# routineLife1/DRBA

Hardware: AMD Instinct MI355X
Metric: interpolated frames/sec @1080p RIFE x2 (higher is better)
Workload: dtype f32 (2xfp16-term MFMA operands = 22 significand bits, fp32 accumulate)

## Files before the change

### drba_amd/_lib.py

```python
import ctypes as C
import os

_HERE = os.path.dirname(os.path.abspath(__file__))
LIB_PATH = os.path.join(_HERE, "csrc", "libdrba_hip.so")
HEADER_PATH = os.path.join(os.path.dirname(_HERE), "include", "drba_hip.h")


def _header_abi_version():
    import re
    if not os.path.exists(HEADER_PATH):
        return None
    with open(HEADER_PATH) as f:
        m = re.search(r"^#define\s+DRBA_ABI_VERSION\s+(\d+)", f.read(), flags=re.M)
    if m is None:
        raise RuntimeError(f"{HEADER_PATH} does not define DRBA_ABI_VERSION")
    return int(m.group(1))


ABI_VERSION = _header_abi_version()

_p = C.c_void_p
_i = C.c_int
_f = C.c_float
_d = C.c_double
# ... 1 lines not shown


class ConvLayer(C.Structure):
    _fields_ = [("packed_w", C.c_void_p), ("bias", C.c_void_p), ("beta", C.c_void_p), ("cin", C.c_int), ("cout", C.c_int),
                ("stride", C.c_int), ("act", C.c_int), ("cfg", C.c_int), ("residual", C.c_int), ("deconv", C.c_int),
                ("pixel_shuffle", C.c_int)]


SIGNATURES = {
    "drba_abi_version": (_i, []),
    "drba_rife_splat_ws_floats": (_z, [_i, _i, _i, _i]),
    "drba_set_range_check": (_i, [_i]),
    "drba_status_word": (_i, [C.POINTER(C.c_void_p)]),
    "drba_status_clear": (_i, []),
    "drba_stream_create_cu_mask": (_i, [C.POINTER(C.c_uint32), _i, C.POINTER(C.c_void_p)]),
    "drba_stream_destroy": (_i, [_p]),
    "drba_conv_state_reset": (_i, [_p]),
    "drba_trace_begin": (_i, []),
    "drba_trace_end": (_i, []),
    "drba_trace_resume": (_i, []),
    "drba_trace_count": (_i, []),
    "drba_trace_get": (_i, [_i, C.POINTER(C.c_char_p), C.POINTER(C.c_uint), C.POINTER(C.c_float)]),
    "drba_trace_get_start": (_i, [_i, C.POINTER(C.c_float), C.POINTER(C.c_ulonglong)]),
    "drba_error_string": (C.c_char_p, [_i]),
    "drba_softsplat": (_i, [_p, _p, _p, _p, _p, _i, _i, _i, _i, _i, _i, _p]),
    "drba_softsplat_ws_floats": (_z, [_i, _i, _i, _i]),
    "drba_softsplat_again": (_i, [_p, _p, _p, _i, _i, _i, _i, _i, _i, _p]),
    "drba_quad_interleave": (_i, [_p, _p, _i, _i, _i, _i, _p]),
    "drba_softsplat_index": (_i, [_p, _p, _p, _i, _i, _i, _i, _p]),
    "drba_softsplat_gather_quad": (_i, [_p, _p, _p, _i, _i, _i, _i, _i, _i, _p]),
    "drba_backwarp": (_i, [_p, _p, _p, _i, _i, _i, _i, _i, _p]),
    "drba_flow_distance": (_i, [_p, _p, _i, _i, _i, _p]),
    "drba_flow_reverse": (_i, [_p, _p, _p, _i, _i, _i, _p]),
    "drba_drm_rife_linear": (_i, [_p, _p, _f, _p, _f, _p, _p, _i, _i, _i, _p]),
    "drba_drm_rife_linear_batch": (_i, [_p, _i, _f, _p, _i, _i, _p]),
    "drba_drm_ratio": (_i, [_p, _p, _f, _p, _p, _i, _i, _i, _p]),
    "drba_affine": (_i, [_p, _f, _f, _p, _z, _p]),
    "drba_mul_map": (_i, [_p, _p, _p, _i, _i, _i, _i, _p]),
    "drba_fill_holes": (_i, [_p, _p, _p, _p, _z, _p]),
    "drba_drm_retime": (_i, [_p, _p, _d, _d, _z, _p]),
    "drba_resize_bilinear": (_i, [_p, _p, _i, _i, _i, _i, _i, _f, _f, _p]),
    "drba_u8hwc_to_f32nchw": (_i, [_p, _p, _i, _i, _p]),
    "drba_f32nchw_to_u8hwc": (_i, [_p, _p, _i, _i, _p]),
    "drba_to_inp": (_i, [_p, _p, _i, _i, _i, _i, _f, _f, _p]),
    "drba_to_inp_x4": (_i, [_p, _p, _p, _i, _i, _i, _i, _f, _f, _p]),
    "drba_to_out": (_i, [_p, _p, _i, _i, _i, _i, _f, _f, _i, _p]),
    "drba_u16hwc_to_f32nchw": (_i, [_p, _p, _i, _i, _f, _p]),
    "drba_f32nchw_to_u16hwc": (_i, [_p, _p, _i, _i, _f, _p]),
    "drba_to_inp16_x4": (_i, [_p, _p, _p, _i, _i, _i, _i, _f, _f, _f, _p]),
    "drba_to_out16": (_i, [_p, _p, _i, _i, _i, _i, _f, _f, _i, _f, _p]),
    "drba_ssim3d_32": (_i, [_p, _p, _p, _p]),
    "drba_ssim3d_ws_floats": (_z, [_i, _i, _i]),
    "drba_ssim3d": (_i, [_p, _p, _p, _p, _i, _i, _i, _i, _d, _p]),
    "drba_frame_error_ws_floats": (_z, [_i, _z]),
    "drba_frame_error_u8": (_i, [_p, _p, _p, _p, _i, _z, _p]),
    "drba_frame_error_f32": (_i, [_p, _p, _p, _p, _i, _z, _p]),
    "drba_frame_error_u16_ws_floats": (_z, [_i, _z]),
    "drba_frame_error_u16": (_i, [_p, _p, _p, _p, _i, _z, _p]),
    "drba_conv3x3_pick_cfg": (_i, [_i, _i, _i, _i, _i]),
    "drba_conv3x3_num_cfgs": (_i, []),
    "drba_conv3x3_cfg_stride": (_i, [_i]),
    "drba_conv3x3_cfg_family": (_i, [_i]),
    "drba_deconv4x4_cfg_family": (_i, [_i]),
    "drba_deconv4x4_num_cfgs": (_i, []),
    "drba_conv3x3_packed_floats": (_z, [_i, _i, _i]),
    "drba_conv3x3_pack": (_i, [_p, _p, _i, _i, _i]),
# ... 126 lines not shown
```

### drba_amd/csrc/common.hpp

```cpp
#pragma once
#include <hip/hip_runtime.h>
#include <hip/hip_ext.h>
#include <stdint.h>
#include <stdlib.h>

#include "../../include/drba_hip.h"

#define DRBA_CHECK_LAUNCH()                                   \
  do {                                                        \
    if (hipGetLastError() != hipSuccess) return DRBA_ELAUNCH; \
  } while (0)

namespace drba {

struct TimedLaunch {
  hipEvent_t start, stop;
};
extern bool g_trace_on;
TimedLaunch trace_launch(const void *host_fn, const char *fallback_name, dim3 grid, hipStream_t stream);

#define DRBA_LAUNCH(kernel, grid, block, lds, stream, ...)                                                     \
  do {                                                                                                         \
    if (drba::g_trace_on) {                                                                                    \
      const drba::TimedLaunch tl_ = drba::trace_launch((const void *)(kernel), #kernel, grid, stream);         \
// ... 172 lines not shown
__device__ __forceinline__ void sample_x4(const float *__restrict__ px, int W, const Taps &t, float (&v)[3]) {
  const int xb = min(t.x0, W - 2);
  const bool edge = t.x0 != xb;
  const f32x4v a0 = *reinterpret_cast<const f32x4v *>(px + ((size_t)t.y0 * W + xb) * 4), a1 = *reinterpret_cast<const f32x4v *>(px + ((size_t)t.y0 * W + xb + 1) * 4);
  const f32x4v b0 = *reinterpret_cast<const f32x4v *>(px + ((size_t)t.y1 * W + xb) * 4), b1 = *reinterpret_cast<const f32x4v *>(px + ((size_t)t.y1 * W + xb + 1) * 4);
#pragma unroll
  for (int c = 0; c < 3; ++c) {
    const float al = edge ? a1[c] : a0[c], bl = edge ? b1[c] : b0[c];
    v[c] = al * t.wnw + a1[c] * t.wne + bl * t.wsw + b1[c] * t.wse;
  }
}

struct Lerp {
  int i0, i1;
  float w0, w1;
};
__device__ __forceinline__ Lerp lerp_src(int dst, float scale, int size) {
  float s = scale * ((float)dst + 0.5f) - 0.5f;
  if (s < 0.f) s = 0.f;
  Lerp l;
  l.i0 = min((int)s, size - 1);
  l.i1 = l.i0 + (l.i0 < size - 1 ? 1 : 0);
  l.w1 = s - (float)l.i0;
  l.w0 = 1.f - l.w1;
  return l;
}

__device__ __forceinline__ float lerp2_fma(float wy0, float wy1, float wx0, float wx1, float p00, float p01, float p10, float p11) {
  const float top = __fmaf_rn(wx0, p00, __fmul_rn(wx1, p01));
  const float bot = __fmaf_rn(wx0, p10, __fmul_rn(wx1, p11));
  return __fmaf_rn(wy0, top, __fmul_rn(wy1, bot));
}

}
```

### drba_amd/csrc/ifnet_glue.hip

```cpp
#include "common.hpp"
#include "flow_terms.hpp"

#include <string.h>

#include <stdlib.h>

using namespace drba;

namespace {

__device__ __forceinline__ Lerp lerp_src_aten(int dst, float scale, int size) {
  float s = __fmaf_rn(scale, (float)dst + 0.5f, -0.5f);
  if (s < 0.f) s = 0.f;
  Lerp l;
  l.i0 = min((int)s, size - 1);
  l.i1 = l.i0 + (l.i0 < size - 1 ? 1 : 0);
  l.w1 = __fsub_rn(s, (float)l.i0);
  l.w0 = __fsub_rn(1.f, l.w1);
  return l;
}
__device__ __forceinline__ float lerp2_aten(const Lerp &ly, const Lerp &lx, float a, float b, float c, float d) {
  const float top = __fmaf_rn(lx.w0, a, __fmul_rn(lx.w1, b));
  const float bot = __fmaf_rn(lx.w0, c, __fmul_rn(lx.w1, d));
  return __fmaf_rn(ly.w0, top, __fmul_rn(ly.w1, bot));
// ... 845 lines not shown
  const float m = 1.f / (1.f + expf(-mk));
  if (img0x) {
    float a[3], b[3];
    sample_x4(img0x, W, t0, a);
    sample_x4(img1x, W, t1, b);
#pragma unroll
    for (int c = 0; c < 3; ++c) out[(size_t)c * P + p] = a[c] * m + b[c] * (1.f - m);
    return;
  }
#pragma unroll
  for (int c = 0; c < 3; ++c) {
    const float a = sample(img0 + (size_t)c * P, W, t0), b = sample(img1 + (size_t)c * P, W, t1);
    out[(size_t)c * P + p] = a * m + b * (1.f - m);
  }
}

__global__ void __launch_bounds__(256)
ifblock_update_kernel(const UpdateItems items, float *__restrict__ mask, float *__restrict__ feat, int h, int w, int H, int W,
                      float scale, float inv_scale) {
  const float *__restrict__ tmp = items.tmp[blockIdx.y];
  const float *flow_in = items.flow_in[blockIdx.y];
  float *flow_out = items.flow_out[blockIdx.y];
  const size_t P = (size_t)H * W, p_lo = (size_t)h * w;
  const int nch = (mask || feat) ? 13 : 4;
  const Tile2D tp_ = tile_pixel(W, H);
  if (tp_.valid) {
    const int y = tp_.y, x = tp_.x;
    const size_t p = (size_t)y * W + x;
    const Lerp ly = lerp_src(y, inv_scale, h), lx = lerp_src(x, inv_scale, w);
    const size_t o00 = (size_t)ly.i0 * w + lx.i0, o01 = (size_t)ly.i0 * w + lx.i1;
    const size_t o10 = (size_t)ly.i1 * w + lx.i0, o11 = (size_t)ly.i1 * w + lx.i1;
    for (int c = 0; c < nch; ++c) {
      const float *t = tmp + (size_t)c * p_lo;
      const float top = lx.w0 * t[o00] + lx.w1 * t[o01];
      const float bot = lx.w0 * t[o10] + lx.w1 * t[o11];
      const float v = ly.w0 * top + ly.w1 * bot;
      if (c < 4) {
        const float fd = v * scale;
        flow_out[(size_t)c * P + p] = flow_in ? flow_in[(size_t)c * P + p] + fd : fd;
      } else if (c == 4) {
        if (mask) mask[p] = v;
      } else if (feat) {
        feat[(size_t)(c - 5) * P + p] = v;
      }
    }
  }
}

__global__ void __launch_bounds__(256)
warp_blend_kernel(const float *__restrict__ img0, const float *__restrict__ img1, const float *__restrict__ flow,
                  const float *__restrict__ mask_lo, int h, int w, float inv_scale, float *__restrict__ out, int H,
                  int W) {
  const size_t P = (size_t)H * W;
  const Tile2D tp_ = tile_pixel(W, H);
  if (tp_.valid) {
    const int y = tp_.y, x = tp_.x;
    const size_t p = (size_t)y * W + x;
    const Taps t0 = taps_border(warp_coord(x, W, flow[p]), warp_coord(y, H, flow[P + p]), W, H);
    const Taps t1 = taps_border(warp_coord(x, W, flow[2 * P + p]), warp_coord(y, H, flow[3 * P + p]), W, H);
    const Lerp ly = lerp_src(y, inv_scale, h), lx = lerp_src(x, inv_scale, w);
    const float top = lx.w0 * mask_lo[(size_t)ly.i0 * w + lx.i0] + lx.w1 * mask_lo[(size_t)ly.i0 * w + lx.i1];
    const float bot = lx.w0 * mask_lo[(size_t)ly.i1 * w + lx.i0] + lx.w1 * mask_lo[(size_t)ly.i1 * w + lx.i1];
    const float mk = ly.w0 * top + ly.w1 * bot;
    const float m = 1.f / (1.f + expf(-mk));
#pragma unroll
    for (int c = 0; c < 3; ++c) {
      const float a = sample(img0 + (size_t)c * P, W, t0), b = sample(img1 + (size_t)c * P, W, t1);
      out[(size_t)c * P + p] = a * m + b * (1.f - m);
    }
  }
}

}
// ... 360 lines not shown
```

### drba_amd/csrc/splat_warp.hip

```cpp
#include "common.hpp"

#include <string.h>

using namespace drba;

namespace {

template <bool ZEROS>
__global__ void __launch_bounds__(256) backwarp_kernel(const float *__restrict__ in, const float *__restrict__ flow,
                                float *__restrict__ out, int C, int H, int W) {
  const int n = blockIdx.y;
  const size_t P = (size_t)H * W;
  in += (size_t)n * C * P;
  flow += (size_t)n * 2 * P;
  out += (size_t)n * C * P;
  for (size_t p = (size_t)blockIdx.x * blockDim.x + threadIdx.x; p < P; p += (size_t)gridDim.x * blockDim.x) {
    const int y = (int)(p / W), x = (int)(p - (size_t)y * W);
    const float sx = warp_coord(x, W, flow[p]), sy = warp_coord(y, H, flow[P + p]);
    if (!ZEROS) {
      const Taps t = taps_border(sx, sy, W, H);
      for (int c = 0; c < C; ++c) out[(size_t)c * P + p] = sample(in + (size_t)c * P, W, t);
    } else {
      const float fx = floorf(sx), fy = floorf(sy);
      const int x0 = (int)fx, y0 = (int)fy;
      const float wx1 = sx - fx, wy1 = sy - fy, wx0 = 1.f - wx1, wy0 = 1.f - wy1;
      const bool okx0 = x0 >= 0 && x0 < W, okx1 = x0 + 1 >= 0 && x0 + 1 < W;
      const bool oky0 = y0 >= 0 && y0 < H, oky1 = y0 + 1 >= 0 && y0 + 1 < H;
      const bool fin = isfinite(sx) && isfinite(sy);
      for (int c = 0; c < C; ++c) {
        const float *pl = in + (size_t)c * P;
        float v = 0.f;
        if (fin) {
          if (okx0 && oky0) v += pl[(size_t)y0 * W + x0] * (wx0 * wy0);
          if (okx1 && oky0) v += pl[(size_t)y0 * W + x0 + 1] * (wx1 * wy0);
// ... 123 lines not shown
    if (x >= W || y >= H) continue;
    const size_t p = (size_t)y * W + x;
    const SplatSrc<MODE> s = splat_source<MODE>(fs, fo, P, p, x, y, t, eps);
    if (!s.finite) continue;
    if (s.is_short) {
      const int rx = s.fx < 0.f ? (int)ceilf(-s.fx) : (int)floorf(s.fx) + 2;
      const int ry = s.fy < 0.f ? (int)ceilf(-s.fy) : (int)floorf(s.fy) + 2;
      r = max(r, max(rx, ry));
      continue;
    }
    if (MODE == 0) {
      const float v[2] = {s.v[0], s.v[1]};
      scatter_avg<2>(gacc, x, y, s.fx, s.fy, v, H, W, dirty, tiles_x);
    } else {
      const float v[1] = {s.v[0]};
      scatter_avg<1>(gacc, x, y, s.fx, s.fy, v, H, W, dirty, tiles_x);
    }
  }
  if ((size_t)gridDim.z * tiles > (size_t)kReachWords) return;
  __shared__ int wr[4];
#pragma unroll
  for (int d = 32; d >= 1; d >>= 1) r = max(r, __shfl_xor(r, d, 64));
  if ((tid & 63) == 0) wr[tid >> 6] = r;
  __syncthreads();
  if (tid == 0) reach[(size_t)n * tiles + blockIdx.y * tiles_x + blockIdx.x] = max(max(wr[0], wr[1]), max(wr[2], wr[3]));
}

constexpr int kSX = 32, kSY = 16;
static_assert(kRMax <= kSY, "the reach map reads the 3 x 3 tiles around an output tile: a halo may not span more than one tile (DRBA_SPLAT_R)");
constexpr int kKX = kSX + 1, kKY = kSY + 1;
constexpr int kNKEY = kKX * kKY;
constexpr int kCAP = 1536;

template <int MODE, int R>
__device__ __forceinline__ void splat_tile_body(const float *__restrict__ fs, const float *__restrict__ fo, float t, float eps,
                                                float *gacc, int *dirty, float *__restrict__ out, int H, int W, int *cnt,
                                                int *wsum, float4 *rec, int *spilled_) {
  constexpr int NV = MODE == 0 ? 2 : 1;
  constexpr int kSWX = kSX + 2 * R, kSWY = kSY + 2 * R;
  constexpr int kSPT = (kSWX * kSWY + 255) / 256;
  constexpr int kR = R;
  volatile int &spilled = *spilled_;
  const size_t P = (size_t)H * W;
  const int was_dirty = __builtin_nontemporal_load(dirty);
  const int tx0 = blockIdx.x * kSX, ty0 = blockIdx.y * kSY;
  const int tid = threadIdx.x;
  for (int i = tid; i <= kNKEY; i += 256) cnt[i] = 0;
  if (tid == 0) spilled = 0;
  __syncthreads();

  float raw[kSPT][MODE == 0 ? 2 : 4];
#pragma unroll
  for (int i = 0; i < kSPT; ++i) {
    const int e = min(tid + i * 256, kSWX * kSWY - 1);
    const int ry = e / kSWX, rx = e - ry * kSWX;
    const int y = min(max(ty0 - kR + ry, 0), H - 1), x = min(max(tx0 - kR + rx, 0), W - 1);
    const size_t p = (size_t)y * W + x;
    raw[i][0] = fs[p];
    raw[i][1] = fs[P + p];
    if (MODE != 0) {
      raw[i][2] = fo[p];
      raw[i][3] = fo[P + p];
    }
  }
  int kr[kSPT];
  float4 val[kSPT];
#pragma unroll
  for (int i = 0; i < kSPT; ++i) {
    kr[i] = -1;
    const int e = tid + i * 256;
    const int ry = e / kSWX, rx = e - ry * kSWX;
    const int y = ty0 - kR + ry, x = tx0 - kR + rx;
    if (e >= kSWX * kSWY || x < 0 || x >= W || y < 0 || y >= H) continue;
    const SplatSrc<MODE> sp = splat_source_from<MODE>(raw[i][0], raw[i][1], MODE == 0 ? 0.f : raw[i][2],
                                                      MODE == 0 ? 0.f : raw[i][3], x, y, t, eps);
    if (!sp.finite || !sp.is_short) continue;
    const float X = (float)x + sp.fx, Y = (float)y + sp.fy;
    const int kx = (int)floorf(X) - tx0 + 1, ky = (int)floorf(Y) - ty0 + 1;
    if (kx < 0 || kx >= kKX || ky < 0 || ky >= kKY) continue;
    const int key = ky * kKX + kx;
    kr[i] = (key << 16) | (atomicAdd(&cnt[key], 1) & 0xFFFF);
    val[i] = make_float4(sp.v[0], sp.v[1], X - (float)tx0, Y - (float)ty0);
  }
  __syncthreads();

  {
    constexpr int PER = (kNKEY + 255) / 256;
    int v[PER], tot = 0;
#pragma unroll
    for (int j = 0; j < PER; ++j) {
      const int k = tid * PER + j;
      v[j] = k < kNKEY ? cnt[k] : 0;
      tot += v[j];
    }
    int inc = tot;
#pragma unroll
    for (int d = 1; d < 64; d <<= 1) {
      const int o = __shfl_up(inc, d, 64);
      if ((tid & 63) >= d) inc += o;
    }
    if ((tid & 63) == 63) wsum[tid >> 6] = inc;
    __syncthreads();
    int run = inc - tot;
    for (int w = 0; w < (tid >> 6); ++w) run += wsum[w];
#pragma unroll
    for (int j = 0; j < PER; ++j) {
// ... 55 lines not shown
        const float wy = dy ? Y - fl_y : (fl_y + 1.f) - Y;
        const float w = wx * wy;
        a0 += r.x * w;
        if (NV == 2) a1 += r.y * w;
        sw += w;
      }
    }
    const size_t p = (size_t)y * W + x;
    float g0 = 0.f, g1 = 0.f, gw = 0.f;
    if (collect) {
      float *g = gacc + p * (NV + 1);
      g0 = g[0], g1 = NV == 2 ? g[1] : 0.f, gw = g[NV];
      if (g0 != 0.f || g1 != 0.f || gw != 0.f) {
        g[0] = 0.f;
        if (NV == 2) g[1] = 0.f;
        g[NV] = 0.f;
      }
    }
    sw += gw;
    const float nrm = sw + 0.0000001f;
    const bool gap = (sw / nrm) < 0.999f;
    if (MODE == 0) {
      a0 += g0;
      a1 += g1;
      out[p] = (gap ? fill : -1.f * (a0 / nrm)) * 2.f;
      out[P + p] = (gap ? fill : -1.f * (a1 / nrm)) * 2.f;
    } else {
      a0 += g0;
      float o = a0 / nrm;
      if (gap) o = splat_source<MODE>(fs, fo, P, p, x, y, t, eps).v[0];
      out[p] = o;
    }
  }
}

template <int MODE>
__global__ void __launch_bounds__(256) splat_tiled(const float *__restrict__ fs, const float *__restrict__ fo, float t,
                                                   const float *__restrict__ t_dev, float eps, float *ws,
                                                   float *__restrict__ out, int H, int W, const SplatJobs jobs) {
  constexpr int NV = MODE == 0 ? 2 : 1;
  if (t_dev) t = *t_dev;
  __shared__ int cnt[kNKEY + 1];
  __shared__ int wsum[4];
  __shared__ float4 rec[kCAP];
  __shared__ int spilled;
  static_assert(kSX == 32 && kSY == 16, "scatter_avg and the pre-pass work on 32 x 16 tiles");
  const int n = blockIdx.z;
  const size_t P = (size_t)H * W;
  if (jobs.n) {
    fs = jobs.fs[n], fo = jobs.fo[n], t = jobs.t[n], out = jobs.out[n];
  } else {
    fs += (size_t)n * 2 * P;
    if (fo) fo += (size_t)n * 2 * P;
    out += (size_t)n * (MODE == 0 ? 2 : 1) * P;
  }
  const int tiles_x = gridDim.x, tiles_y = gridDim.y, tiles = tiles_x * tiles_y;
  const int *reach = reinterpret_cast<const int *>(ws) + (size_t)n * tiles;
  float *gacc = ws + kReachWords;
  int *dirty = reinterpret_cast<int *>(gacc + (size_t)gridDim.z * P * (NV + 1)) + ((size_t)n * tiles_y + blockIdx.y) * tiles_x + blockIdx.x;
  gacc += (size_t)n * P * (NV + 1);
  int r = kRMax;
  if ((size_t)gridDim.z * tiles <= (size_t)kReachWords) {
    r = 0;
    const int bx = blockIdx.x, by = blockIdx.y;
#pragma unroll
    for (int dy = -1; dy <= 1; ++dy)
#pragma unroll
      for (int dx = -1; dx <= 1; ++dx) {
        const int yy = by + dy, xx = bx + dx;
        if (yy >= 0 && yy < tiles_y && xx >= 0 && xx < tiles_x) r = max(r, __builtin_nontemporal_load(reach + yy * tiles_x + xx));
      }
    r = __builtin_amdgcn_readfirstlane(r);
  }
  if (r <= 4) splat_tile_body<MODE, 4>(fs, fo, t, eps, gacc, dirty, out, H, W, cnt, wsum, rec, &spilled);
  else if (r <= 8) splat_tile_body<MODE, 8>(fs, fo, t, eps, gacc, dirty, out, H, W, cnt, wsum, rec, &spilled);
  else splat_tile_body<MODE, kRMax>(fs, fo, t, eps, gacc, dirty, out, H, W, cnt, wsum, rec, &spilled);
}


constexpr int kChunk = 16, kScanPerBlock = 4096;

struct __attribute__((aligned(16))) SplatRec {
  int src;
  float X, Y;
  float m;
};

__device__ __forceinline__ float splat_weight_1d(float X, float fl, int d) { return d ? X - fl : (fl + 1.f) - X; }

__device__ __forceinline__ long long splat_key(const float *__restrict__ flow, size_t P, size_t p, int x, int y, int H, int W,
                                               float &X, float &Y) {
  X = (float)x + flow[p];
  Y = (float)y + flow[P + p];
  if (!(isfinite(X) && isfinite(Y))) return -1;
  const float fx = floorf(X), fy = floorf(Y);
  if (fx < -1.f || fx > (float)(W - 1) || fy < -1.f || fy > (float)(H - 1)) return -1;
  return (long long)((int)fy + 1) * (W + 1) + ((int)fx + 1);
}

__global__ void __launch_bounds__(256) splat_sort_count(const float *__restrict__ flow, int *__restrict__ cnt, int H, int W) {
  const int n = blockIdx.y;
  const size_t P = (size_t)H * W, Pk = (size_t)(H + 1) * (W + 1);
  flow += (size_t)n * 2 * P;
  cnt += (size_t)n * Pk;
  for (size_t p = (size_t)blockIdx.x * blockDim.x + threadIdx.x; p < P; p += (size_t)gridDim.x * blockDim.x) {
    const int y = (int)(p / W), x = (int)(p - (size_t)y * W);
    float X, Y;
    const long long k = splat_key(flow, P, p, x, y, H, W, X, Y);
    if (k >= 0) atomicAdd(&cnt[k], 1);
// ... 350 lines not shown
  else
    DRBA_LAUNCH(backwarp_kernel<true>, g, dim3(kBlock), 0, (hipStream_t)stream, in, flow, out, C, H, W);
  DRBA_CHECK_LAUNCH();
  return DRBA_OK;
}

int drba_flow_distance(const float *flow, float *out, int N, int H, int W, void *stream) {
  if (!flow || !out || N <= 0 || H <= 0 || W <= 0) return DRBA_EINVAL;
  dim3 g(grid_for((size_t)H * W), N);
  DRBA_LAUNCH(distance_kernel, g, dim3(kBlock), 0, (hipStream_t)stream, flow, out, H, W);
  DRBA_CHECK_LAUNCH();
  return DRBA_OK;
}

size_t drba_rife_splat_ws_floats(int N, int H, int W, int values) {
  if (N <= 0 || H <= 0 || W <= 0 || values < 1 || values > 2) return 0;
  return (size_t)kReachWords + (size_t)N * H * W * (values + 1) + (size_t)N * ((W + kSX - 1) / kSX) * ((H + kSY - 1) / kSY);
}

int drba_flow_reverse(const float *flow, float *out, float *ws, int N, int H, int W, void *stream) {
  if (!flow || !out || !ws || N <= 0 || H <= 0 || W <= 0) return DRBA_EINVAL;
  hipStream_t s = (hipStream_t)stream;
  SplatJobs none;
  none.n = 0;
  dim3 g((W + kSX - 1) / kSX, (H + kSY - 1) / kSY, N);
  DRBA_LAUNCH(splat_long_prepass<0>, g, dim3(kBlock), 0, s, flow, (const float *)nullptr, 0.f,
                     (const float *)nullptr, 0.f, ws, H, W, none);
  DRBA_LAUNCH(splat_tiled<0>, g, dim3(kBlock), 0, s, flow, (const float *)nullptr, 0.f, (const float *)nullptr,
                     0.f, ws, out, H, W, none);
  DRBA_CHECK_LAUNCH();
  return DRBA_OK;
}

int drba_drm_rife_linear(const float *flow_self, const float *flow_other, float t, const float *t_dev, float eps,
                         float *out, float *ws, int N, int H, int W, void *stream) {
  if (!flow_self || !flow_other || !out || !ws || N <= 0 || H <= 0 || W <= 0) return DRBA_EINVAL;
  hipStream_t s = (hipStream_t)stream;
  SplatJobs none;
  none.n = 0;
  dim3 g((W + kSX - 1) / kSX, (H + kSY - 1) / kSY, N);
  DRBA_LAUNCH(splat_long_prepass<1>, g, dim3(kBlock), 0, s, flow_self, flow_other, t, t_dev,
                     eps, ws, H, W, none);
  DRBA_LAUNCH(splat_tiled<1>, g, dim3(kBlock), 0, s, flow_self, flow_other, t, t_dev, eps, ws, out, H, W, none);
  DRBA_CHECK_LAUNCH();
  return DRBA_OK;
}

int drba_drm_rife_linear_batch(const drba_drm_job_t *jobs, int n_jobs, float eps, float *ws, int H, int W, void *stream) {
  if (!jobs || n_jobs <= 0 || n_jobs > DRBA_MAX_STAGE_ITEMS || !ws || H <= 0 || W <= 0) return DRBA_EINVAL;
  SplatJobs J;
  memset(&J, 0, sizeof(J));
  J.n = n_jobs;
  for (int k = 0; k < n_jobs; ++k) {
    if (!jobs[k].flow_self || !jobs[k].flow_other || !jobs[k].out) return DRBA_EINVAL;
    J.fs[k] = jobs[k].flow_self, J.fo[k] = jobs[k].flow_other, J.t[k] = jobs[k].t, J.out[k] = jobs[k].out;
  }
  hipStream_t s = (hipStream_t)stream;
  dim3 g((W + kSX - 1) / kSX, (H + kSY - 1) / kSY, n_jobs);
  DRBA_LAUNCH(splat_long_prepass<1>, g, dim3(kBlock), 0, s, J.fs[0], J.fo[0], 0.f, (const float *)nullptr, eps, ws,
              H, W, J);
  DRBA_LAUNCH(splat_tiled<1>, g, dim3(kBlock), 0, s, J.fs[0], J.fo[0], 0.f, (const float *)nullptr, eps, ws, J.out[0], H, W, J);
  DRBA_CHECK_LAUNCH();
  return DRBA_OK;
}

int drba_drm_ratio(const float *flow10, const float *flow12, float eps, float *drm10, float *drm12, int N, int H,
// ... 39 lines not shown
```

### drba_amd/models/rife.py

```python
import os

import numpy as np
import torch

from drba_amd import handoff, ops as _ops
from drba_amd.models.lookahead import Lookahead, shared_stream
from drba_amd.models.lookahead import split as split_lookahead
from drba_amd.models.drm import calc_drm_rife
from drba_amd.models.rife_426_heavy.IFNet_HDv3 import IFNet
from drba_amd.models.utils.tools import convert, load_weights


class RIFE:
    supports_lookahead = True
    STAT_KEYS = ("groups_formed", "staged_groups", "group_collects", "groups_dropped", "single_steps", "encoder_prefetch_hits",
                 "encoder_prefetch_misses", "pairflow_prefetch_hits", "lookahead_hits")
    stats = None

    def _count(self, key):
        if self.stats is None:
            self.stats = dict.fromkeys(self.STAT_KEYS, 0)
        self.stats[key] += 1
    _look = None

# ... 30 lines not shown
                if f0 is None:
                    f0, f1 = self._encoded(I0), self._encoded(I1)
                output.append(len(items))
                items.append((I0, I1, float(t), f0, f1))
        return self._fill(output, items)

    def _fill(self, output, items):
        if items:
            frames = self.ifnet.forward_pairs(items, self.scale_list)
            output = [frames[o] if isinstance(o, int) else o for o in output]
        return output

    def calc_flow(self, a, b, f0=None, f1=None):
        _, _, H, W = a.shape
        f0 = self._encoded(a) if f0 is None else f0
        f1 = self._encoded(b) if f1 is None else f1
        s = self.scale_list[0]
        xin = _ops.ifblock_input(a, b, f0, f1, 0.5, None, None, 1.0, s)
        flow = _ops.ifblock_update(self.ifnet.block[0].core(xin), None, H, W, s)
        rev = _ops.flow_reverse(flow.reshape(2, 2, H, W))
        flow01, flow10 = rev[0:1], rev[1:2]
        if _ops.PAIR_FEATURES and f0.is_cuda:
            _ops.pair_interleaved(f0)
            _ops.pair_interleaved(f1)
        return flow01, flow10, f0, f1

    def calc_flow_batch(self, pairs):
        B = len(pairs)
        _, _, H, W = pairs[0][0].shape
        s = self.scale_list[0]
        h, w = int(np.floor(H * (1.0 / s))), int(np.floor(W * (1.0 / s)))
        xin = torch.empty((B, 39, h, w), dtype=torch.float32, device=pairs[0][0].device)
        _ops.stage_inputs([(a, b, 0.5, fa, fb) for a, b, fa, fb in pairs], None, None, 1.0, s, xin, lds=False)
        flow = _ops.flow_updates(self.ifnet.block[0].core(xin), [None] * B, H, W, s, whole=True)
        rev = _ops.flow_reverse(flow.reshape(2 * B, 2, H, W))
        out = []
        for k, (a, b, fa, fb) in enumerate(pairs):
            if _ops.PAIR_FEATURES:
                _ops.pair_interleaved(fa)
                _ops.pair_interleaved(fb)
            out.append((rev[2 * k:2 * k + 1], rev[2 * k + 1:2 * k + 2], fa, fb))
        return out

    def _group_flows(self, F, n, fa):
        P, todo = [None] * n, []
        for j in range(n):
            a, b = F[j + 1], F[j + 2]
            if handoff.peek(b, "_drba_pairflow", handoff.token_of(self), a) is not None:
                P[j] = self._pair_flow(a, b, None)
            else:
                todo.append(j)
        if todo:
            feats = {}
            for j in todo:
                for x in (F[j + 1], F[j + 2]):
                    if id(x) not in feats:
                        feats[id(x)] = fa if (x is F[1] and fa is not None) else self._encoded(x)
            res = self.calc_flow_batch([(F[j + 1], F[j + 2], feats[id(F[j + 1])], feats[id(F[j + 2])]) for j in todo])
            for j, r in zip(todo, res):
                P[j] = r
        return P

    def intake_stream(self, device):
        if self.ENC_ON_MAIN:
            return None
        if getattr(self, "_enc_stream", None) is None:
            self._enc_stream = shared_stream(device, "prefetch")
        return self._enc_stream
# ... 207 lines not shown
```

### drba_amd/ops.py

```python
import ctypes as C
import math
import os

import numpy as np
import torch

from drba_amd import _lib
from drba_amd import tunecache as _tunecache

_MODES = {"sum": 0, "avg": 1, "linear": 2, "soft": 3}
_EPS = {None: 0, "addeps": 0, "zeroeps": 1, "clipeps": 2}


def default_device():
    if not torch.cuda.is_available():
        raise _lib.DrbaHipError("drba_amd needs an MI355X (no GPU visible and there is no CPU fallback)")
    return torch.device("cuda", torch.cuda.current_device())


_raw_stream = getattr(torch._C, "_cuda_getCurrentRawStream", None)


def _stream():
    if _raw_stream is not None:
# ... 213 lines not shown
                       "drba_softsplat_again")
        res.append(out)
    return res


def backwarp(x, flow, padding="border"):
    x, flow = _f32(x, "input"), _f32(flow, "flow")
    n, c, h, w = x.shape
    out = torch.empty_like(x)
    _lib.check(_lib.load().drba_backwarp(_p(x), _p(flow), _p(out), n, c, h, w, 0 if padding == "border" else 1,
                                         _stream()), "drba_backwarp")
    return out


def flow_distance(flow):
    flow = _f32(flow, "flow")
    n, _, h, w = flow.shape
    out = torch.empty((n, 1, h, w), dtype=torch.float32, device=flow.device)
    _lib.check(_lib.load().drba_flow_distance(_p(flow), _p(out), n, h, w, _stream()), "drba_flow_distance")
    return out


def flow_reverse(flow):
    flow = _f32(flow, "flow")
    n, _, h, w = flow.shape
    out = torch.empty_like(flow)
    ws = _zero_workspace(flow.device, _lib.load().drba_rife_splat_ws_floats(n, h, w, 2))
    first = _trace_pos()
    _lib.check(_lib.load().drba_flow_reverse(_p(flow), _p(out), _p(ws), n, h, w, _stream()), "drba_flow_reverse")
    _tag(first, [None, (16.0 * n * h * w, "byte", f"flow_reverse {(n, h, w)}")])
    return out


def drm_rife_linear(flow_self, flow_other, t, eps=1e-4, t_dev=None):
    a, b = _f32(flow_self, "flow_self"), _f32(flow_other, "flow_other")
    n, _, h, w = a.shape
    out = torch.empty((n, 1, h, w), dtype=torch.float32, device=a.device)
    ws = _zero_workspace(a.device, _lib.load().drba_rife_splat_ws_floats(n, h, w, 1))
    first = _trace_pos()
    _lib.check(_lib.load().drba_drm_rife_linear(_p(a), _p(b), float(t), _p(t_dev), float(eps), _p(out), _p(ws), n, h,
                                                w, _stream()), "drba_drm_rife_linear")
    _tag(first, [None, (20.0 * n * h * w, "byte", f"drm_rife_linear {(n, h, w)}")])
    return out


def drm_rife_linear_many(jobs, eps=1e-4):
    if not jobs:
        return []
    flows = [(_f32(a, "flow_self"), _f32(b, "flow_other"), float(t)) for a, b, t in jobs]
    _, _, h, w = flows[0][0].shape
    dev = flows[0][0].device
    res = []
    for c0 in range(0, len(flows), _lib.MAX_STAGE_ITEMS):
        chunk = flows[c0:c0 + _lib.MAX_STAGE_ITEMS]
        n = len(chunk)
        out = torch.empty((n, 1, h, w), dtype=torch.float32, device=dev)
        arr = (_lib.DrmJob * n)()
        for k, (a, b, t) in enumerate(chunk):
            if tuple(a.shape) != (1, 2, h, w) or tuple(b.shape) != (1, 2, h, w):
                raise _lib.DrbaHipError("drm_rife_linear_many: every flow must be [1,2,H,W] of one size")
            arr[k].flow_self, arr[k].flow_other, arr[k].t, arr[k].out = a.data_ptr(), b.data_ptr(), t, out[k].data_ptr()
        ws = _zero_workspace(dev, _lib.load().drba_rife_splat_ws_floats(n, h, w, 1))
        first = _trace_pos()
        _lib.check(_lib.load().drba_drm_rife_linear_batch(C.cast(arr, C.c_void_p), n, float(eps), _p(ws), h, w, _stream()),
                   "drba_drm_rife_linear_batch")
        _tag(first, [None, (20.0 * n * h * w, "byte", f"drm_rife_linear {(n, h, w)}")])
# ... 1258 lines not shown
```

### include/drba_hip.h

```cpp
#ifndef DRBA_HIP_H
#define DRBA_HIP_H

#include <stddef.h>
#include <stdint.h>

#ifdef __cplusplus
extern "C" {
#endif

#define DRBA_OK 0
#define DRBA_EINVAL (-1)
#define DRBA_EUNSUPPORTED (-2)
#define DRBA_ELAUNCH (-3)

#define DRBA_ABI_VERSION 12
int drba_abi_version(void);
const char *drba_error_string(int code);
int drba_set_range_check(int on);
#define DRBA_STATUS_CONV_SPLIT 0
#define DRBA_STATUS_CONV_DMA 1
#define DRBA_STATUS_CONV_KS 2
#define DRBA_STATUS_LINEAR 3
#define DRBA_STATUS_ATTENTION 4
#define DRBA_STATUS_STAGE 5
#define DRBA_STATUS_HEAD 6
int drba_status_word(volatile unsigned long long **host_word);
int drba_status_clear(void);

int drba_conv_state_reset(void *stream);
int drba_stream_create_cu_mask(const uint32_t *mask, int words, void **stream);
int drba_stream_destroy(void *stream);

int drba_trace_begin(void);
int drba_trace_end(void);
int drba_trace_resume(void);
int drba_trace_count(void);
int drba_trace_get(int i, const char **name, unsigned *grid3, float *ms);
int drba_trace_get_start(int i, float *ms_since_first, unsigned long long *stream);

int drba_softsplat(const float *in, const float *flow, const float *metric, float *out, float *ws,
                   int N, int C, int H, int W, int mode, int eps, void *stream);
size_t drba_softsplat_ws_floats(int N, int C, int H, int W);
int drba_softsplat_again(const float *in, float *out, float *ws, int N, int C, int H, int W, int mode, int eps, void *stream);
int drba_quad_interleave(const float *in, float *out, int N, int C, int H, int W, void *stream);
int drba_softsplat_index(const float *flow, const float *metric, float *ws, int N, int H, int W, int mode, void *stream);
int drba_softsplat_gather_quad(const float *in_quad, float *out, float *ws, int N, int C, int H, int W, int mode, int eps,
                               void *stream);

int drba_backwarp(const float *in, const float *flow, float *out, int N, int C, int H, int W,
                  int padding, void *stream);

int drba_flow_distance(const float *flow, float *out, int N, int H, int W, void *stream);

size_t drba_rife_splat_ws_floats(int N, int H, int W, int values);
int drba_flow_reverse(const float *flow, float *out, float *ws, int N, int H, int W, void *stream);

int drba_drm_rife_linear(const float *flow_self, const float *flow_other, float t, const float *t_dev,
                         float eps, float *out, float *ws, int N, int H, int W, void *stream);
typedef struct drba_drm_job {
  const float *flow_self, *flow_other;
  float t;
  float *out;
} drba_drm_job_t;
int drba_drm_rife_linear_batch(const drba_drm_job_t *jobs, int n_jobs, float eps, float *ws, int H, int W, void *stream);

int drba_drm_ratio(const float *flow10, const float *flow12, float eps, float *drm10, float *drm12,
                   int N, int H, int W, void *stream);
int drba_affine(const float *a, float mul, float add, float *out, size_t n, void *stream);
int drba_mul_map(const float *x, const float *map, float *out, int N, int C, int H, int W, void *stream);
int drba_fill_holes(const float *aligned, const float *cover, const float *value, float *out,
                    size_t n, void *stream);
int drba_drm_retime(const float *drm, float *out, double t, double precision, size_t n, void *stream);

int drba_resize_bilinear(const float *in, float *out, int NC, int Hin, int Win, int Hout, int Wout,
                         float scale_y, float scale_x, void *stream);
int drba_u8hwc_to_f32nchw(const uint8_t *in, float *out, int H, int W, void *stream);
int drba_f32nchw_to_u8hwc(const float *in, uint8_t *out, int H, int W, void *stream);
int drba_to_inp(const uint8_t *img_hwc, float *out, int Hin, int Win, int Hout, int Wout, float scale_y, float scale_x,
                void *stream);
int drba_to_inp_x4(const uint8_t *img_hwc, float *out, float *out_x4, int Hin, int Win, int Hout, int Wout, float scale_y,
                   float scale_x, void *stream);
int drba_to_out(const float *in, uint8_t *out_hwc, int Hin, int Win, int Hout, int Wout, float scale_y, float scale_x,
                int reverse_channels, void *stream);
int drba_u16hwc_to_f32nchw(const uint16_t *in, float *out, int H, int W, float maxval, void *stream);
int drba_f32nchw_to_u16hwc(const float *in, uint16_t *out, int H, int W, float maxval, void *stream);
int drba_to_inp16_x4(const uint16_t *img_hwc, float *out, float *out_x4, int Hin, int Win, int Hout, int Wout, float scale_y,
                     float scale_x, float maxval, void *stream);
int drba_to_out16(const float *in, uint16_t *out_hwc, int Hin, int Win, int Hout, int Wout, float scale_y, float scale_x,
// ... 160 lines not shown
```

Before: 1233.

## Fuse head flow upsampling into flow reversal splatting via LDS footprint

Adds a fused path that reads the low-resolution IFNet head output directly and bilinearly upsamples the flow inside the splat tile kernel, using an LDS footprint and per-row/column tables. This avoids materializing the full-resolution flow and re-reading it in the separate flow-reversal pass. A prepass computes per-tile reach from the low-res bounds and only scatters long-range sources when needed. The head-flow rounding is shared through a common helper so results match the old path. It falls back to the old path when the scale or batch size is unsupported.

```diff
diff --git a/drba_amd/_lib.py b/drba_amd/_lib.py
--- a/drba_amd/_lib.py
+++ b/drba_amd/_lib.py
@@ -57,6 +57,7 @@
     "drba_backwarp": (_i, [_p, _p, _p, _i, _i, _i, _i, _i, _p]),
     "drba_flow_distance": (_i, [_p, _p, _i, _i, _i, _p]),
     "drba_flow_reverse": (_i, [_p, _p, _p, _i, _i, _i, _p]),
+    "drba_flow_reverse_head_batch": (_i, [_p, _i, _i, _i, _i, _i, _f, _p, _p, _p, _p]),
     "drba_drm_rife_linear": (_i, [_p, _p, _f, _p, _f, _p, _p, _i, _i, _i, _p]),
     "drba_drm_rife_linear_batch": (_i, [_p, _i, _f, _p, _i, _i, _p]),
     "drba_drm_ratio": (_i, [_p, _p, _f, _p, _p, _i, _i, _i, _p]),
diff --git a/drba_amd/csrc/common.hpp b/drba_amd/csrc/common.hpp
--- a/drba_amd/csrc/common.hpp
+++ b/drba_amd/csrc/common.hpp
@@ -228,4 +228,9 @@
   return __fmaf_rn(wy0, top, __fmul_rn(wy1, bot));
 }
 
-}
+__device__ __forceinline__ float head_flow(float wy0, float wy1, float wx0, float wx1, float p00, float p01, float p10, float p11,
+                                           float scale) {
+  return __fmul_rn(lerp2_fma(wy0, wy1, wx0, wx1, p00, p01, p10, p11), scale);
+}
+
+}
diff --git a/drba_amd/csrc/ifnet_glue.hip b/drba_amd/csrc/ifnet_glue.hip
--- a/drba_amd/csrc/ifnet_glue.hip
+++ b/drba_amd/csrc/ifnet_glue.hip
@@ -901,13 +901,15 @@
     const size_t o10 = (size_t)ly.i1 * w + lx.i0, o11 = (size_t)ly.i1 * w + lx.i1;
     for (int c = 0; c < nch; ++c) {
       const float *t = tmp + (size_t)c * p_lo;
+      if (c < 4) {
+        const float fd = head_flow(ly.w0, ly.w1, lx.w0, lx.w1, t[o00], t[o01], t[o10], t[o11], scale);
+        flow_out[(size_t)c * P + p] = flow_in ? flow_in[(size_t)c * P + p] + fd : fd;
+        continue;
+      }
       const float top = lx.w0 * t[o00] + lx.w1 * t[o01];
       const float bot = lx.w0 * t[o10] + lx.w1 * t[o11];
       const float v = ly.w0 * top + ly.w1 * bot;
-      if (c < 4) {
-        const float fd = v * scale;
-        flow_out[(size_t)c * P + p] = flow_in ? flow_in[(size_t)c * P + p] + fd : fd;
-      } else if (c == 4) {
+      if (c == 4) {
         if (mask) mask[p] = v;
       } else if (feat) {
         feat[(size_t)(c - 5) * P + p] = v;
diff --git a/drba_amd/csrc/splat_warp.hip b/drba_amd/csrc/splat_warp.hip
--- a/drba_amd/csrc/splat_warp.hip
+++ b/drba_amd/csrc/splat_warp.hip
@@ -1,5 +1,6 @@
 #include "common.hpp"
 
+#include <float.h>
 #include <string.h>
 
 using namespace drba;
@@ -189,10 +190,27 @@
 constexpr int kNKEY = kKX * kKY;
 constexpr int kCAP = 1536;
 
-template <int MODE, int R>
+struct HeadFlows {
+  const float *tmp[DRBA_MAX_STAGE_ITEMS];
+  int h, w;
+  float scale, inv_scale;
+  float *flow_out;
+};
+constexpr int kHeadC = 12, kHeadR = 10;
+struct HeadTile {
+  const float *hd;
+  float2 *foot;
+  int2 *colt, *rowt;
+  float *flow_out;
+  int h, w;
+  float scale, inv_scale;
+};
+
+template <int MODE, int R, bool HEAD = false>
 __device__ __forceinline__ void splat_tile_body(const float *__restrict__ fs, const float *__restrict__ fo, float t, float eps,
                                                 float *gacc, int *dirty, float *__restrict__ out, int H, int W, int *cnt,
-                                                int *wsum, float4 *rec, int *spilled_) {
+                                                int *wsum, float4 *rec, int *spilled_, const HeadTile *ht = nullptr) {
+  static_assert(!HEAD || MODE == 0, "only the flow reversal forms its sources from a head output");
   constexpr int NV = MODE == 0 ? 2 : 1;
   constexpr int kSWX = kSX + 2 * R, kSWY = kSY + 2 * R;
   constexpr int kSPT = (kSWX * kSWY + 255) / 256;
@@ -204,6 +222,26 @@
   const int tid = threadIdx.x;
   for (int i = tid; i <= kNKEY; i += 256) cnt[i] = 0;
   if (tid == 0) spilled = 0;
+  if (HEAD) {
+    const int h = ht->h, w = ht->w;
+    const float inv = ht->inv_scale;
+    const int xa = max(tx0 - kR, 0), xb = min(tx0 + kSX + kR - 1, W - 1), ya = max(ty0 - kR, 0), yb = min(ty0 + kSY + kR - 1, H - 1);
+    const int cx0 = lerp_src(xa, inv, w).i0, cy0 = lerp_src(ya, inv, h).i0;
+    const int ncol = min(lerp_src(xb, inv, w).i1 - cx0 + 1, kHeadC), nrow = min(lerp_src(yb, inv, h).i1 - cy0 + 1, kHeadR);
+    static_assert(kHeadC * kHeadR <= 256 && kSX + 2 * kRMax <= 64 && 64 + kSY + 2 * kRMax <= 256, "one footprint sample / table entry per thread");
+    if (tid < nrow * ncol) {
+      const int r = tid / ncol, c = tid - r * ncol;
+      const size_t o = (size_t)(cy0 + r) * w + (cx0 + c);
+      ht->foot[r * kHeadC + c] = make_float2(ht->hd[o], ht->hd[(size_t)h * w + o]);
+    }
+    if (tid < kSWX) {
+      const Lerp l = lerp_src(min(max(tx0 - kR + tid, 0), W - 1), inv, w);
+      ht->colt[tid] = make_int2(min(l.i0 - cx0, kHeadC - 1) | (min(l.i1 - cx0, kHeadC - 1) << 16), __float_as_int(l.w1));
+    } else if (tid >= 64 && tid < 64 + kSWY) {
+      const Lerp l = lerp_src(min(max(ty0 - kR + tid - 64, 0), H - 1), inv, h);
+      ht->rowt[tid - 64] = make_int2((min(l.i0 - cy0, kHeadR - 1) * kHeadC) | ((min(l.i1 - cy0, kHeadR - 1) * kHeadC) << 16), __float_as_int(l.w1));
+    }
+  }
   __syncthreads();
 
   float raw[kSPT][MODE == 0 ? 2 : 4];
@@ -211,6 +249,7 @@
   for (int i = 0; i < kSPT; ++i) {
     const int e = min(tid + i * 256, kSWX * kSWY - 1);
     const int ry = e / kSWX, rx = e - ry * kSWX;
+    if (HEAD) continue;
     const int y = min(max(ty0 - kR + ry, 0), H - 1), x = min(max(tx0 - kR + rx, 0), W - 1);
     const size_t p = (size_t)y * W + x;
     raw[i][0] = fs[p];
@@ -229,6 +268,19 @@
     const int ry = e / kSWX, rx = e - ry * kSWX;
     const int y = ty0 - kR + ry, x = tx0 - kR + rx;
     if (e >= kSWX * kSWY || x < 0 || x >= W || y < 0 || y >= H) continue;
+    if (HEAD) {
+      const int2 ct = ht->colt[rx], rt = ht->rowt[ry];
+      const float wx1 = __int_as_float(ct.y), wy1 = __int_as_float(rt.y);
+      const float wx0 = 1.f - wx1, wy0 = 1.f - wy1;
+      const float2 q00 = ht->foot[(rt.x & 0xFFFF) + (ct.x & 0xFFFF)], q01 = ht->foot[(rt.x & 0xFFFF) + (ct.x >> 16)];
+      const float2 q10 = ht->foot[(rt.x >> 16) + (ct.x & 0xFFFF)], q11 = ht->foot[(rt.x >> 16) + (ct.x >> 16)];
+      raw[i][0] = head_flow(wy0, wy1, wx0, wx1, q00.x, q01.x, q10.x, q11.x, ht->scale);
+      raw[i][1] = head_flow(wy0, wy1, wx0, wx1, q00.y, q01.y, q10.y, q11.y, ht->scale);
+      if (ht->flow_out && rx >= kR && rx < kR + kSX && ry >= kR && ry < kR + kSY) {
+        ht->flow_out[(size_t)y * W + x] = raw[i][0];
+        ht->flow_out[P + (size_t)y * W + x] = raw[i][1];
+      }
+    }
     const SplatSrc<MODE> sp = splat_source_from<MODE>(raw[i][0], raw[i][1], MODE == 0 ? 0.f : raw[i][2],
                                                       MODE == 0 ? 0.f : raw[i][3], x, y, t, eps);
     if (!sp.finite || !sp.is_short) continue;
@@ -350,6 +402,22 @@
       out[p] = o;
     }
   }
+}
+
+__device__ __forceinline__ int splat_tile_halo(const float *ws) {
+  const int tiles_x = gridDim.x, tiles_y = gridDim.y, tiles = tiles_x * tiles_y;
+  if ((size_t)gridDim.z * tiles > (size_t)kReachWords) return kRMax;
+  const int *reach = reinterpret_cast<const int *>(ws) + (size_t)blockIdx.z * tiles;
+  int r = 0;
+  const int bx = blockIdx.x, by = blockIdx.y;
+#pragma unroll
+  for (int dy = -1; dy <= 1; ++dy)
+#pragma unroll
+    for (int dx = -1; dx <= 1; ++dx) {
+      const int yy = by + dy, xx = bx + dx;
+      if (yy >= 0 && yy < tiles_y && xx >= 0 && xx < tiles_x) r = max(r, __builtin_nontemporal_load(reach + yy * tiles_x + xx));
+    }
+  return __builtin_amdgcn_readfirstlane(r);
 }
 
 template <int MODE>
@@ -372,27 +440,116 @@
     if (fo) fo += (size_t)n * 2 * P;
     out += (size_t)n * (MODE == 0 ? 2 : 1) * P;
   }
-  const int tiles_x = gridDim.x, tiles_y = gridDim.y, tiles = tiles_x * tiles_y;
-  const int *reach = reinterpret_cast<const int *>(ws) + (size_t)n * tiles;
+  const int tiles_x = gridDim.x, tiles_y = gridDim.y;
   float *gacc = ws + kReachWords;
   int *dirty = reinterpret_cast<int *>(gacc + (size_t)gridDim.z * P * (NV + 1)) + ((size_t)n * tiles_y + blockIdx.y) * tiles_x + blockIdx.x;
   gacc += (size_t)n * P * (NV + 1);
-  int r = kRMax;
-  if ((size_t)gridDim.z * tiles <= (size_t)kReachWords) {
-    r = 0;
-    const int bx = blockIdx.x, by = blockIdx.y;
-#pragma unroll
-    for (int dy = -1; dy <= 1; ++dy)
-#pragma unroll
-      for (int dx = -1; dx <= 1; ++dx) {
-        const int yy = by + dy, xx = bx + dx;
-        if (yy >= 0 && yy < tiles_y && xx >= 0 && xx < tiles_x) r = max(r, __builtin_nontemporal_load(reach + yy * tiles_x + xx));
-      }
-    r = __builtin_amdgcn_readfirstlane(r);
-  }
+  const int r = splat_tile_halo(ws);
   if (r <= 4) splat_tile_body<MODE, 4>(fs, fo, t, eps, gacc, dirty, out, H, W, cnt, wsum, rec, &spilled);
   else if (r <= 8) splat_tile_body<MODE, 8>(fs, fo, t, eps, gacc, dirty, out, H, W, cnt, wsum, rec, &spilled);
   else splat_tile_body<MODE, kRMax>(fs, fo, t, eps, gacc, dirty, out, H, W, cnt, wsum, rec, &spilled);
+}
+
+__global__ void __launch_bounds__(64) splat_head_prepass(const HeadFlows hf, float *__restrict__ ws, int H, int W) {
+  const int n = blockIdx.z, lane = threadIdx.x;
+  const int h = hf.h, w = hf.w;
+  const size_t P = (size_t)H * W, p_lo = (size_t)h * w;
+  const float *__restrict__ hd = hf.tmp[n >> 1] + (size_t)(n & 1) * 2 * p_lo;
+  const int tiles_x = gridDim.x, tiles = tiles_x * gridDim.y;
+  const bool have_map = (size_t)gridDim.z * tiles <= (size_t)kReachWords;
+  int *reach = reinterpret_cast<int *>(ws) + (size_t)n * tiles + blockIdx.y * tiles_x + blockIdx.x;
+  const int x0 = blockIdx.x * kSX, y0 = blockIdx.y * kSY;
+  const int cx0 = lerp_src(x0, hf.inv_scale, w).i0, cy0 = lerp_src(y0, hf.inv_scale, h).i0;
+  const int nc = lerp_src(min(x0 + kSX - 1, W - 1), hf.inv_scale, w).i1 - cx0 + 1;
+  const int ns = nc * (lerp_src(min(y0 + kSY - 1, H - 1), hf.inv_scale, h).i1 - cy0 + 1);
+  float lo[2] = {INFINITY, INFINITY}, hi[2] = {-INFINITY, -INFINITY};
+  int fin = 1;
+  for (int e = lane; e < ns; e += 64) {
+    const int r = e / nc, c = e - r * nc;
+    const size_t o = (size_t)(cy0 + r) * w + (cx0 + c);
+    const float v[2] = {hd[o], hd[p_lo + o]};
+#pragma unroll
+    for (int k = 0; k < 2; ++k) {
+      fin &= isfinite(v[k]) ? 1 : 0;
+      lo[k] = fminf(lo[k], v[k]);
+      hi[k] = fmaxf(hi[k], v[k]);
+    }
+  }
+#pragma unroll
+  for (int d = 32; d >= 1; d >>= 1) {
+    fin &= __shfl_xor(fin, d, 64);
+#pragma unroll
+    for (int k = 0; k < 2; ++k) {
+      lo[k] = fminf(lo[k], __shfl_xor(lo[k], d, 64));
+      hi[k] = fmaxf(hi[k], __shfl_xor(hi[k], d, 64));
+    }
+  }
+  int rb = 0;
+  bool all_short = fin != 0;
+#pragma unroll
+  for (int k = 0; k < 2; ++k) {
+    const float m = fmaxf(fabsf(lo[k]), fabsf(hi[k])) * hf.scale * 0x1p-20f + FLT_MIN;
+    const float L = lo[k] * hf.scale - m, U = hi[k] * hf.scale + m;
+    all_short = all_short && L >= -(float)kRMax && U < (float)(kRMax - 1);
+    if (all_short) rb = max(rb, max(L < 0.f ? (int)ceilf(-L) : 0, U >= 0.f ? (int)floorf(U) + 2 : 0));
+  }
+  if (all_short) {
+    if (have_map && lane == 0) *reach = rb;
+    return;
+  }
+  float *gacc = ws + kReachWords;
+  int *dirty = reinterpret_cast<int *>(gacc + (size_t)gridDim.z * P * 3) + (size_t)n * tiles;
+  gacc += (size_t)n * P * 3;
+  int r = 0;
+  for (int i = 0; i < kSX * kSY / 64; ++i) {
+    const int x = x0 + (lane & 31), y = y0 + (lane >> 5) + 2 * i;
+    if (x >= W || y >= H) continue;
+    const Lerp ly = lerp_src(y, hf.inv_scale, h), lx = lerp_src(x, hf.inv_scale, w);
+    const size_t o00 = (size_t)ly.i0 * w + lx.i0, o01 = (size_t)ly.i0 * w + lx.i1;
+    const size_t o10 = (size_t)ly.i1 * w + lx.i0, o11 = (size_t)ly.i1 * w + lx.i1;
+    const float su = head_flow(ly.w0, ly.w1, lx.w0, lx.w1, hd[o00], hd[o01], hd[o10], hd[o11], hf.scale);
+    const float sv = head_flow(ly.w0, ly.w1, lx.w0, lx.w1, hd[p_lo + o00], hd[p_lo + o01], hd[p_lo + o10], hd[p_lo + o11], hf.scale);
+    const SplatSrc<0> s = splat_source_from<0>(su, sv, 0.f, 0.f, x, y, 0.f, 0.f);
+    if (!s.finite) continue;
+    if (s.is_short) {
+      const int rx = s.fx < 0.f ? (int)ceilf(-s.fx) : (int)floorf(s.fx) + 2;
+      const int ry = s.fy < 0.f ? (int)ceilf(-s.fy) : (int)floorf(s.fy) + 2;
+      r = max(r, max(rx, ry));
+      continue;
+    }
+    const float v[2] = {s.v[0], s.v[1]};
+    scatter_avg<2>(gacc, x, y, s.fx, s.fy, v, H, W, dirty, tiles_x);
+  }
+  if (!have_map) return;
+#pragma unroll
+  for (int d = 32; d >= 1; d >>= 1) r = max(r, __shfl_xor(r, d, 64));
+  if (lane == 0) *reach = r;
+}
+
+__global__ void __launch_bounds__(256) splat_tiled_head(const HeadFlows hf, float *ws, float *__restrict__ out, int H, int W) {
+  __shared__ int cnt[kNKEY + 1];
+  __shared__ int wsum[4];
+  __shared__ float4 rec[kCAP];
+  __shared__ int spilled;
+  float2 *foot = reinterpret_cast<float2 *>(rec);
+  int2 *colt = reinterpret_cast<int2 *>(foot + kHeadR * kHeadC), *rowt = colt + (kSX + 2 * kRMax);
+  static_assert((kHeadR * kHeadC + kSX + kSY + 4 * kRMax) * 8 <= kCAP * 16, "footprint and tables fit the record space");
+  const int n = blockIdx.z;
+  const size_t P = (size_t)H * W;
+  out += (size_t)n * 2 * P;
+  const int tiles_x = gridDim.x, tiles_y = gridDim.y;
+  float *gacc = ws + kReachWords;
+  int *dirty = reinterpret_cast<int *>(gacc + (size_t)gridDim.z * P * 3) + ((size_t)n * tiles_y + blockIdx.y) * tiles_x + blockIdx.x;
+  gacc += (size_t)n * P * 3;
+  HeadTile ht;
+  ht.hd = hf.tmp[n >> 1] + (size_t)(n & 1) * 2 * hf.h * hf.w;
+  ht.foot = foot, ht.colt = colt, ht.rowt = rowt;
+  ht.flow_out = hf.flow_out ? hf.flow_out + (size_t)n * 2 * P : nullptr;
+  ht.h = hf.h, ht.w = hf.w, ht.scale = hf.scale, ht.inv_scale = hf.inv_scale;
+  const int r = splat_tile_halo(ws);
+  if (r <= 4) splat_tile_body<0, 4, true>(nullptr, nullptr, 0.f, 0.f, gacc, dirty, out, H, W, cnt, wsum, rec, &spilled, &ht);
+  else if (r <= 8) splat_tile_body<0, 8, true>(nullptr, nullptr, 0.f, 0.f, gacc, dirty, out, H, W, cnt, wsum, rec, &spilled, &ht);
+  else splat_tile_body<0, kRMax, true>(nullptr, nullptr, 0.f, 0.f, gacc, dirty, out, H, W, cnt, wsum, rec, &spilled, &ht);
 }
 
 
@@ -809,6 +966,25 @@
   return DRBA_OK;
 }
 
+int drba_flow_reverse_head_batch(const float *const *tmp, int n, int h, int w, int H, int W, float scale, float *out, float *ws,
+                                 float *flow_out, void *stream) {
+  if (!tmp || !out || !ws || n <= 0 || n > DRBA_MAX_STAGE_ITEMS || h <= 0 || w <= 0 || H <= 0 || W <= 0 || !(scale > 0.f)) return DRBA_EINVAL;
+  HeadFlows hf;
+  memset(&hf, 0, sizeof(hf));
+  for (int k = 0; k < n; ++k) {
+    if (!tmp[k]) return DRBA_EINVAL;
+    hf.tmp[k] = tmp[k];
+  }
+  hf.h = h, hf.w = w, hf.scale = scale, hf.inv_scale = (float)(1.0 / (double)scale), hf.flow_out = flow_out;
+  if (!((double)(kSX + 2 * kRMax) / scale + 3.0 <= kHeadC && (double)(kSY + 2 * kRMax) / scale + 3.0 <= kHeadR)) return DRBA_EUNSUPPORTED;
+  hipStream_t s = (hipStream_t)stream;
+  dim3 g((W + kSX - 1) / kSX, (H + kSY - 1) / kSY, 2 * n);
+  DRBA_LAUNCH(splat_head_prepass, g, dim3(64), 0, s, hf, ws, H, W);
+  DRBA_LAUNCH(splat_tiled_head, g, dim3(kBlock), 0, s, hf, ws, out, H, W);
+  DRBA_CHECK_LAUNCH();
+  return DRBA_OK;
+}
+
 int drba_drm_rife_linear(const float *flow_self, const float *flow_other, float t, const float *t_dev, float eps,
                          float *out, float *ws, int N, int H, int W, void *stream) {
   if (!flow_self || !flow_other || !out || !ws || N <= 0 || H <= 0 || W <= 0) return DRBA_EINVAL;
diff --git a/drba_amd/models/rife.py b/drba_amd/models/rife.py
--- a/drba_amd/models/rife.py
+++ b/drba_amd/models/rife.py
@@ -86,8 +86,11 @@
         h, w = int(np.floor(H * (1.0 / s))), int(np.floor(W * (1.0 / s)))
         xin = torch.empty((B, 39, h, w), dtype=torch.float32, device=pairs[0][0].device)
         _ops.stage_inputs([(a, b, 0.5, fa, fb) for a, b, fa, fb in pairs], None, None, 1.0, s, xin, lds=False)
-        flow = _ops.flow_updates(self.ifnet.block[0].core(xin), [None] * B, H, W, s, whole=True)
-        rev = _ops.flow_reverse(flow.reshape(2 * B, 2, H, W))
+        tmp = self.ifnet.block[0].core(xin)
+        rev = _ops.flow_reverse_head(tmp, H, W, s)
+        if rev is None:
+            flow = _ops.flow_updates(tmp, [None] * B, H, W, s, whole=True)
+            rev = _ops.flow_reverse(flow.reshape(2 * B, 2, H, W))
         out = []
         for k, (a, b, fa, fb) in enumerate(pairs):
             if _ops.PAIR_FEATURES:
diff --git a/drba_amd/ops.py b/drba_amd/ops.py
--- a/drba_amd/ops.py
+++ b/drba_amd/ops.py
@@ -269,6 +269,27 @@
     return out
 
 
+def flow_reverse_head(tmp, H, W, scale, want_flow=False):
+    tmp = _f32(tmp, "tmp")
+    B, c, h, w = tmp.shape
+    if c < 4:
+        raise _lib.DrbaHipError(f"flow_reverse_head: tmp must be [B, >= 4, h, w], got {tuple(tmp.shape)}")
+    if B > _lib.MAX_STAGE_ITEMS:
+        return None
+    out = torch.empty((2 * B, 2, H, W), dtype=torch.float32, device=tmp.device)
+    flow = torch.empty((B, 4, H, W), dtype=torch.float32, device=tmp.device) if want_flow else None
+    a_tmp = (C.c_void_p * B)(*[tmp[k].data_ptr() for k in range(B)])
+    ws = _zero_workspace(tmp.device, _lib.load().drba_rife_splat_ws_floats(2 * B, H, W, 2))
+    first = _trace_pos()
+    code = _lib.load().drba_flow_reverse_head_batch(C.cast(a_tmp, C.c_void_p), B, h, w, H, W, float(scale), _p(out), _p(ws),
+                                                    _p(flow), _stream())
+    if code == _EUNSUPPORTED:
+        return None
+    _lib.check(code, "drba_flow_reverse_head_batch")
+    _tag(first, [None, (4.0 * B * (4.0 * H * W + 4.0 * h * w), "byte", f"flow_reverse_head {(B, h, w, H, W)}")])
+    return (out, flow) if want_flow else out
+
+
 def drm_rife_linear(flow_self, flow_other, t, eps=1e-4, t_dev=None):
     a, b = _f32(flow_self, "flow_self"), _f32(flow_other, "flow_other")
     n, _, h, w = a.shape
diff --git a/include/drba_hip.h b/include/drba_hip.h
--- a/include/drba_hip.h
+++ b/include/drba_hip.h
@@ -13,7 +13,7 @@
 #define DRBA_EUNSUPPORTED (-2)
 #define DRBA_ELAUNCH (-3)
 
-#define DRBA_ABI_VERSION 12
+#define DRBA_ABI_VERSION 13
 int drba_abi_version(void);
 const char *drba_error_string(int code);
 int drba_set_range_check(int on);
@@ -54,6 +54,8 @@
 
 size_t drba_rife_splat_ws_floats(int N, int H, int W, int values);
 int drba_flow_reverse(const float *flow, float *out, float *ws, int N, int H, int W, void *stream);
+int drba_flow_reverse_head_batch(const float *const *tmp, int n, int h, int w, int H, int W, float scale, float *out, float *ws,
+                                 float *flow_out, void *stream);
 
 int drba_drm_rife_linear(const float *flow_self, const float *flow_other, float t, const float *t_dev,
                          float eps, float *out, float *ws, int N, int H, int W, void *stream);
```

Result: no change. 1245, median of 6 (+0.9%).
